# Geo3DSmart/PDANet

Hardware: AMD Instinct MI355X
Metric: scenes/sec (16384-pt ONCE, PDA-SSD forward+backward) (higher is better)
Workload: dtype f32; 1 GPU; once16k_b2_detector_fwd_bwd_adam; scenes_per_gpu=2, global_batch=2, parallelism=dp1, world_size_seen=1, cpu_affinity=GPU-local NUMA node of 0000:dc:00.0: 128 CPUs, full=False, graph_tail=False, graph_head=True

## Files before the change

include/pda_train.h:

```cpp
#ifndef PDA_TRAIN_H
#define PDA_TRAIN_H
#include "pda_pointnet2.h"

#ifdef __cplusplus
extern "C" {
#endif

int pda_grad_norm(const float *g, int64_t n, float *norm_out, float *scratch1024, pda_stream_t stream);
int pda_adam_onecycle_step(float *p, const float *g, float *m, float *v, int64_t n, float lr,
                           float beta1, float beta2, float eps, float wd, int step,
                           const float *total_norm, float max_norm, pda_stream_t stream);

int64_t pda_bn_relu_scratch_bytes(int c);
int pda_bn_relu_fwd(const float *x, const float *gamma, const float *beta, float *running_mean,
                    float *running_var, float *y, float *mean_invstd, void *scratch, int64_t rows, int c,
                    float eps, float momentum, pda_stream_t stream);
int pda_bn_relu_bwd(const float *x, const float *grad_y, const float *gamma, const float *beta,
                    const float *mean_invstd, float *grad_x, float *grad_gamma, float *grad_beta,
                    void *scratch, int64_t rows, int c, pda_stream_t stream);
int pda_bn_relu_fwd_counted(const float *x, const float *gamma, const float *beta, float *running_mean, float *running_var,
                            float *y, float *mean_invstd, void *scratch, int64_t rows, int c, float eps, float momentum,
                            const int32_t *count, int32_t *status, int relu, int training, pda_stream_t stream);
int pda_bn_relu_bwd_counted(const float *x, const float *grad_y, const float *gamma, const float *beta,
                            const float *mean_invstd, float *grad_x, float *grad_gamma, float *grad_beta, void *scratch,
// ... 203 lines not shown
int pda_nms_bev(const float *boxes, const int32_t *num_valid, int64_t *keep, int32_t *num_keep,
                uint64_t *mask_scratch, int b, int n, float thresh, int normal, pda_stream_t stream);
int pda_multi_nms_compact(const float *boxes, const float *scores, const int64_t *keep, const int32_t *num_keep,
                          const int32_t *label_map, int b, int c, int k, int post_max, float *pred_boxes, float *pred_scores,
                          int64_t *pred_labels, int32_t *num_pred, pda_stream_t stream);
int pda_multi_nms_compact_wide(int box_cols, const float *boxes, const float *scores, const int64_t *keep,
                               const int32_t *num_keep, const int32_t *label_map, int b, int c, int k, int post_max,
                               float *pred_boxes, float *pred_scores, int64_t *pred_labels, int32_t *num_pred,
                               pda_stream_t stream);

int pda_head_cls_loss(const float *preds, int row_stride, int col0, int num_class, const int64_t *labels, const float *soft,
                      int64_t n, float scale, float *out2, float *grad, pda_stream_t stream);
int pda_head_centerness(const float *centers, const float *gt, const int64_t *labels, float *out, int64_t n, pda_stream_t stream);
int pda_head_box_loss(const float *preds, const float *labels, const int64_t *cls_labels, const float *code_weights, float beta,
                      int bins, float dir_weight, float box_weight, int64_t n, float *out4, float *grad, pda_stream_t stream);
int pda_head_vote_loss(int mode, const float *origin, const float *offsets, const int64_t *key, const float *gt, int b, int boxes,
                       int num_class, float weight, int64_t n, float *out1, float *grad, pda_stream_t stream);
int pda_head_corner_loss(const float *box_preds, const float *centers, const float *cls_preds, int num_class, const float *gt,
                         const int64_t *cls_labels, const float *mean_size, int bins, float weight, int64_t n, float *out1,
                         float *grad_box, float *grad_centers, pda_stream_t stream);

int64_t pda_sa_small_train_workspace_bytes(void);
int pda_sa_small_train_supported(int c, int nsample, int c1, int c2, int c3, int64_t tokens);
int pda_sa_small_train_fwd(const float *xyz, const float *new_xyz, const float *feat_pm, const int32_t *idx,
                           const float *w1, const float *w2, const float *w3, const float *const *gamma,
                           const float *const *beta, float *const *running_mean, float *const *running_var,
                           const float *eps, const float *momentum, void *workspace, float *out, float *zmax,
                           uint8_t *arg, int b, int n, int m, int c, int nsample, int c1, int c2, int c3,
                           pda_stream_t stream);
int pda_sa_small_train_bwd(const float *xyz, const float *new_xyz, const float *feat_pm, const int32_t *idx,
                           const float *grad_out, const float *zmax, const uint8_t *arg, void *workspace, float *dz2,
                           float *dz1, float *dw1, float *dw2, float *dw3, float *const *dgamma, float *const *dbeta,
                           int b, int n, int m, int c, int nsample, int c1, int c2, int c3, pda_stream_t stream);

int64_t pda_sa_xyz_grad_scratch_bytes(int c1);
int pda_sa_point_gather(const float *point_rows, const float *xyz, const float *new_xyz, const int32_t *idx, const float *w,
                        int ldw, const float *bias, int relu, float *z, int b, int n, int m, int nsample, int c1,
                        pda_stream_t stream);
int pda_sa_xyz_grad(const float *grad_z1, const float *xyz, const float *new_xyz, const int32_t *idx, const float *w, int ldw,
                    float *dw, int lddw, float *grad_new_xyz, void *scratch, int b, int n, int m, int nsample, int c1,
                    pda_stream_t stream);
int64_t pda_sa_point_gather_stats_blocks(int64_t tokens, int c1);
int pda_sa_point_gather_stats(const float *point_rows, const float *xyz, const float *new_xyz, const int32_t *idx,
                              const float *w, int ldw, float *z, double *partial, int b, int n, int m, int nsample, int c1,
                              pda_stream_t stream);
int pda_sa_point_grad_bn(const float *grad_a1, const float *z1, const float *mean_invstd, const float *gamma,
                         const float *beta, const float *bwd_sums, const float *xyz, const float *new_xyz, const int32_t *idx,
                         const float *w, int ldw, float *dw, int lddw, float *grad_new_xyz, float *grad_points, void *scratch,
                         int b, int n, int m, int nsample, int c1, pda_stream_t stream);

int64_t pda_input_stage_workspace_bytes(int batch, int64_t n_cap);
int pda_input_stage(const float *points, const int64_t *offsets, int64_t n_total, int batch, int c, int64_t n_cap,
                    const float *range6, int num_points, const int32_t *pick, const int32_t *perm1, const int32_t *perm2,
                    uint64_t seed, int shuffle, float *out_points, int32_t *info, void *workspace, pda_stream_t stream);
int pda_input_boxes(const float *boxes, const int64_t *box_offsets, int64_t m_total, int batch, int box_dim, int max_gt,
                    const float *range6, int min_num_corners, float *gt_boxes, int32_t *info, pda_stream_t stream);

int64_t pda_augment_workspace_bytes(int batch, int64_t n_cap, int k);
int pda_augment(const float *points, const int64_t *offsets, int64_t n_total, int batch, int c, int64_t n_cap,
                const float *boxes, const int64_t *box_offsets, int64_t m_total, const float *db_points,
                const int64_t *db_offsets, int64_t db_n_points, const float *db_boxes, const double *db_centre,
                const int32_t *db_class, int n_obj, const int32_t *cand, const int32_t *cand_group, const double *cand_dz,
                int k, const int32_t *flip, const double *angle, const float *scale, const float *remove_extra_width,
                int64_t paste_cap, float *out_points, int64_t out_cap, int64_t *out_offsets, float *out_boxes,
                int64_t out_box_cap, int64_t *out_box_offsets, int32_t *info, void *workspace, pda_stream_t stream);

// ... 323 lines not shown
```

pdanet_amd/_lib.py:

```python
import ctypes
import os

_HERE = os.path.dirname(os.path.abspath(__file__))
LIB_PATH = os.environ.get("PDA_LIB_PATH") or os.path.join(_HERE, "libpda_pointnet2.so")
ABI_VERSION = 20


class DensityNetScale(ctypes.Structure):
    _fields_ = [("x", ctypes.c_void_p), ("grad_y", ctypes.c_void_p), ("params", ctypes.c_void_p), ("y", ctypes.c_void_p),
                ("stats", ctypes.c_void_p), ("scratch", ctypes.c_void_p), ("running", ctypes.c_void_p * 6),
                ("grad_params", ctypes.c_void_p), ("n", ctypes.c_int64), ("rowmap", ctypes.c_void_p),
                ("row_weight", ctypes.c_void_p), ("n_unique", ctypes.c_void_p), ("nsample", ctypes.c_int),
                ("eps", ctypes.c_float), ("momentum", ctypes.c_float)]


class OnceFrames(ctypes.Structure):
    _fields_ = [("gt_boxes", ctypes.c_void_p), ("gt_name", ctypes.c_void_p), ("gt_offsets", ctypes.c_void_p),
                ("pred_boxes", ctypes.c_void_p), ("pred_score", ctypes.c_void_p), ("pred_name", ctypes.c_void_p),
                ("pred_start", ctypes.c_void_p), ("pred_count", ctypes.c_void_p), ("iou_start", ctypes.c_void_p),
                ("n_gt_total", ctypes.c_int64), ("pred_cap", ctypes.c_int64), ("iou_cap", ctypes.c_int64),
                ("n_frames", ctypes.c_int), ("max_gt", ctypes.c_int), ("max_pred", ctypes.c_int)]


class KittiFrames(ctypes.Structure):
# ... 105 lines not shown
    "pda_densitynet_param_count": [],
    "pda_densitynet_eval_param_count": [],
    "pda_densitynet_scratch_bytes": [],
    "pda_densitynet_fwd": [_vp, _vp, _vp, _vp, _vp, _vp, _vp, _vp, _vp, _vp, _vp, ctypes.c_int64, _f, _f, _vp],
    "pda_densitynet_bwd": [_vp, _vp, _vp, _vp, _vp, _vp, ctypes.c_int64, _f, _vp],
    "pda_densitynet_eval": [_vp, _vp, _vp, ctypes.c_int64, _vp],
    "pda_densitynet_fwd_multi": [_vp, _i, _vp],
    "pda_densitynet_bwd_multi": [_vp, _i, _vp],
    "pda_densitynet_fwd_unique": [_vp, _vp, _vp, _vp, _vp, _vp, _vp, _vp, _vp, _vp, _vp, ctypes.c_int64, _vp, _vp, _vp, _i, _f, _f, _vp],
    "pda_densitynet_bwd_unique": [_vp, _vp, _vp, _vp, _vp, _vp, ctypes.c_int64, _vp, _vp, _vp, _i, _f, _vp],
    "pda_pda_geometry": [_vp, _vp, _vp, _vp, _vp, _i, _i, _i, _i, _f, _vp],
    "pda_points_in_boxes": [_vp, _vp, _vp, _i, _i, _i, _vp],
    "pda_roiaware_pool3d_fwd": [_vp, _vp, _vp, _vp, _vp, _vp, _i, _i, _i, _i, _i, _i, _i, _i, _vp],
    "pda_roiaware_pool3d_bwd": [_vp, _vp, _vp, _vp, _i, _i, _i, _i, _i, _i, _i, _i, _vp],
    "pda_roipoint_pool3d_fwd": [_vp, _vp, _vp, _vp, _vp, _i, _i, _i, _i, _i, _vp],
    "pda_points_in_boxes_mask": [_vp, _vp, _vp, _i, _i, _vp],
    "pda_points_in_boxes_count": [_vp, _i, _vp, _vp, _i, _i, _i, _vp],
    "pda_assign_point_targets": [_vp, _vp, _vp, _vp, _vp, _vp, _i, _i, _i, _i, _i, _vp],
    "pda_sa_gaussian_mask": [_vp, _i, _i, _vp, _vp, _vp, ctypes.c_int64, _vp],
    "pda_head_assign_targets": [_vp, _i, _i, _vp, ctypes.POINTER(ctypes.c_float), _vp, _vp, _vp, _vp, _vp, _i, _i, _i, _i, _i, _i, _vp],
    "pda_head_cls_loss": [_vp, _i, _i, _i, _vp, _vp, ctypes.c_int64, _f, _vp, _vp, _vp],
    "pda_head_centerness": [_vp, _vp, _vp, _vp, ctypes.c_int64, _vp],
    "pda_head_box_loss": [_vp, _vp, _vp, _vp, _f, _i, _f, _f, ctypes.c_int64, _vp, _vp, _vp],
    "pda_head_vote_loss": [_i, _vp, _vp, _vp, _vp, _i, _i, _i, _f, ctypes.c_int64, _vp, _vp, _vp],
    "pda_head_corner_loss": [_vp, _vp, _vp, _i, _vp, _vp, _vp, _i, _f, ctypes.c_int64, _vp, _vp, _vp, _vp],
    "pda_boxes_overlap_bev": [_vp, _vp, _vp, _i, _i, _vp],
    "pda_boxes_iou_bev": [_vp, _vp, _vp, _i, _i, _vp],
    "pda_nms_mask_words": [_i],
    "pda_nms_bev": [_vp, _vp, _vp, _vp, _vp, _i, _i, _f, _i, _vp],
    "pda_sa_small_train_workspace_bytes": [],
    "pda_sa_small_train_supported": [_i, _i, _i, _i, _i, ctypes.c_int64],
    "pda_sa_small_train_fwd": [_vp] * 7 + [ctypes.POINTER(_vp)] * 4 + [ctypes.POINTER(_f)] * 2 + [_vp] * 4 + [_i] * 8 + [_vp],
    "pda_sa_small_train_bwd": [_vp] * 13 + [ctypes.POINTER(_vp)] * 2 + [_i] * 8 + [_vp],
    "pda_sa_xyz_grad_scratch_bytes": [_i],
    "pda_sa_point_gather": [_vp, _vp, _vp, _vp, _vp, _i, _vp, _i, _vp, _i, _i, _i, _i, _i, _vp],
    "pda_sa_xyz_grad": [_vp, _vp, _vp, _vp, _vp, _i, _vp, _i, _vp, _vp, _i, _i, _i, _i, _i, _vp],
    "pda_sa_point_gather_stats_blocks": [ctypes.c_int64, _i],
    "pda_sa_point_gather_stats": [_vp, _vp, _vp, _vp, _vp, _i, _vp, _vp, _i, _i, _i, _i, _i, _vp],
    "pda_sa_point_grad_bn": [_vp] * 10 + [_i, _vp, _i, _vp, _vp, _vp, _i, _i, _i, _i, _i, _vp],
    "pda_adam_onecycle_step": [_vp, _vp, _vp, _vp, ctypes.c_int64, _f, _f, _f, _f, _f, _i, _vp, _f, _vp],
    "pda_input_stage_workspace_bytes": [_i, ctypes.c_int64],
    "pda_input_stage": [_vp, _vp, ctypes.c_int64, _i, _i, ctypes.c_int64, ctypes.POINTER(_f), _i, _vp, _vp, _vp,
                        ctypes.c_uint64, _i, _vp, _vp, _vp, _vp],
    "pda_input_boxes": [_vp, _vp, ctypes.c_int64, _i, _i, _i, ctypes.POINTER(_f), _i, _vp, _vp, _vp],
    "pda_augment_workspace_bytes": [_i, ctypes.c_int64, _i],
    "pda_augment": [_vp, _vp, ctypes.c_int64, _i, _i, ctypes.c_int64, _vp, _vp, ctypes.c_int64, _vp, _vp, ctypes.c_int64, _vp,
                    _vp, _vp, _i, _vp, _vp, _vp, _i, _vp, _vp, _vp, ctypes.POINTER(_f), ctypes.c_int64, _vp, ctypes.c_int64,
                    _vp, _vp, ctypes.c_int64, _vp, _vp, _vp, _vp],
    "pda_augment_paste": [_vp, _vp, ctypes.c_int64, _i, _i, ctypes.c_int64, _vp, _vp, ctypes.c_int64, _vp, _vp, ctypes.c_int64, _vp,
                          _vp, _vp, _i, _vp, _vp, _vp, _i, ctypes.POINTER(_f), ctypes.c_int64, _vp, ctypes.c_int64, _vp, _vp,
                          ctypes.c_int64, _vp, _vp, _vp, _vp],
    "pda_augment_steps_workspace_bytes": [_i, ctypes.c_int64, _i, _i],
    "pda_augment_steps": [_vp, _vp, ctypes.c_int64, _i, _i, ctypes.c_int64, _vp, _vp, ctypes.c_int64,
                          ctypes.POINTER(ctypes.c_int32), _i, _vp, _vp, _i, _i, _vp, _vp, ctypes.c_int64, _vp, _vp,
                          ctypes.c_int64, _vp, _vp, _vp, _vp],
    "pda_pyramid_aug_workspace_bytes": [_i, ctypes.c_int64, _i],
    "pda_pyramid_aug": [_vp, _vp, ctypes.c_int64, _i, _i, ctypes.c_int64, _vp, _vp, ctypes.c_int64, _vp, _vp, _vp, _vp, _vp, _i,
                        ctypes.POINTER(ctypes.c_double), _i, _i, _i, _vp, _vp, ctypes.c_int64, _vp, _vp, ctypes.c_int64, _vp,
                        _vp, _vp, _vp],
    "pda_once_eval_workspace_bytes": [_i, ctypes.c_int64, _i],
    "pda_once_eval_iou": [ctypes.POINTER(OnceFrames), _i, _vp, _vp, _vp],
    "pda_once_eval_accumulate": [ctypes.POINTER(OnceFrames), _vp, _vp, _i, _i, ctypes.POINTER(ctypes.c_double), _i, _vp, _vp,
                                 _vp, _vp],
    "pda_once_eval_match": [ctypes.POINTER(OnceFrames), _vp, _vp, _i, _i, ctypes.POINTER(ctypes.c_double), _i, _i, _vp, _vp,
                            _vp, _vp, _vp, _vp, _vp, _vp],
    "pda_kitti_eval_workspace_bytes": [_i, ctypes.c_int64, ctypes.c_int64, _i],
# ... 183 lines not shown
```

pdanet_amd/csrc/sa_train_small.hip:

```cpp
#include "pda_common.h"

namespace pda {

typedef float f32x16 __attribute__((ext_vector_type(16)));

constexpr int SS_WAVES = 8;
constexpr int SS_LD = 33;
constexpr int SS_LDS_WAVE = 96 * SS_LD;
constexpr int SS_LDS_WPACK = 6400;
constexpr int SS_LDS_STATE = 768;
__host__ __device__ constexpr int ss_lds_floats(int waves) { return SS_LDS_WPACK + SS_LDS_STATE + waves * SS_LDS_WAVE; }
constexpr int SS_MAX_BLOCKS = 512;
constexpr int SS_PART = 128;
constexpr int SS_DW = 2048;
__host__ __device__ constexpr int ss_state_base(int layer) { return (layer - 1) * 192; }
static_assert(384 + 6 * 64 <= 1024, "the state (floats) fits the first 4 KB of the workspace");
__host__ __device__ constexpr int ss_off_w2() { return 256; }
__host__ __device__ constexpr int ss_off_w3() { return 256 + 1024; }
__host__ __device__ constexpr int ss_off_w2t(int R3) { return 256 + 1024 + 1024 * R3; }
__host__ __device__ constexpr int ss_off_w3t(int R3) { return 256 + 2048 + 1024 * R3; }
__host__ __device__ constexpr int ss_wpack_floats(int R3) { return 256 + 2048 + 2048 * R3; }

struct SsParams {
    const float* xyz;
    const float* new_xyz;
    const float* feat;
    const int32_t* idx;
    const float* wpack;
    const float* state;
    double* partial;
    float* out;
    float* zmax;
    uint8_t* arg;
    const float* gout;
    const uint8_t* arg_in;
    float* dz_out;
    const float* dz_in;
    float* dw_partial;
    int n, m, c, ns, c1, c2, c3;
    int64_t tiles;
};

__device__ __forceinline__ float ss_pack_one(const float* __restrict__ w, int o, int rows, int cols, int R, int mode, int trans) {
    const int e = o & 3, lane = (o >> 2) & 63, rest = o >> 8;
    const int rb = rest % R, tq = rest / R;
    const int t = tq * 4 + e, h = lane >> 5;
    const int row = rb * 32 + (lane & 31);
    int k;
    if (mode == 0) k = 2 * t + h;
    else { const int tt = t & 15; k = 32 * (t >> 4) + (tt & 3) + 8 * (tt >> 2) + 4 * h; }
    if (row >= rows || k >= cols) return 0.f;
    return trans ? w[(size_t)k * rows + row] : w[(size_t)row * cols + k];
}

__global__ void ss_pack_kernel(const float* __restrict__ w1, const float* __restrict__ w2, const float* __restrict__ w3,
                               float* __restrict__ wpack, int c0, int c1, int c2, int c3, int R3) {
    const int total = ss_wpack_floats(R3);
    for (int o = blockIdx.x * blockDim.x + threadIdx.x; o < total; o += gridDim.x * blockDim.x) {
        float v;
        if (o < ss_off_w2()) v = ss_pack_one(w1, o, c1, c0, 1, 0, 0);
        else if (o < ss_off_w3()) v = ss_pack_one(w2, o - ss_off_w2(), c2, c1, 1, 1, 0);
        else if (o < ss_off_w2t(R3)) v = ss_pack_one(w3, o - ss_off_w3(), c3, c2, R3, 1, 0);
        else if (o < ss_off_w3t(R3)) v = ss_pack_one(w2, o - ss_off_w2t(R3), c1, c2, 1, 1, 1);
        else v = ss_pack_one(w3, o - ss_off_w3t(R3), c2, c3, 1, 1, 1);
        wpack[o] = v;
    }
}

template <int KS, int R>
struct SsFrag {
    const float* wf;
    int lane;
    __device__ __forceinline__ void load(const float* lds_wf, int l) { wf = lds_wf; lane = l; }
    __device__ __forceinline__ float4 f(int tq, int r) const { return *reinterpret_cast<const float4*>(wf + ((tq * R + r) * 64 + lane) * 4); }
};

template <int KS, int R, typename HinT>
__device__ __forceinline__ void ss_mm(f32x16 (&acc)[R], const HinT& hin, const SsFrag<KS, R>& w) {
#pragma unroll
    for (int r = 0; r < R; ++r)
#pragma unroll
        for (int i = 0; i < 16; ++i) acc[r][i] = 0.f;
#pragma unroll
    for (int tq = 0; tq < KS / 4; ++tq)
#pragma unroll
        for (int e = 0; e < 4; ++e) {
            const float b = hin(tq * 4 + e);
#pragma unroll
            for (int r = 0; r < R; ++r) {
                const float4 a4 = w.f(tq, r);
// ... 150 lines not shown
    }
}

__device__ __forceinline__ void ss_to_lds(float* __restrict__ t, const f32x16& v, int rb, int lane) {
    const int h = lane >> 5, j = lane & 31;
#pragma unroll
    for (int i = 0; i < 16; ++i) t[(rb * 32 + (i & 3) + 8 * (i >> 2) + 4 * h) * SS_LD + j] = v[i];
}

template <int NB>
__device__ __forceinline__ void ss_dw_tile(f32x16 (&dw)[NB], const float* __restrict__ zt, const float* __restrict__ yt, int lane) {
    const int h = lane >> 5, c = lane & 31;
#pragma unroll
    for (int t = 0; t < 16; ++t) {
        if ((t & 3) == 0) __builtin_amdgcn_sched_barrier(0);
        const float b = yt[c * SS_LD + 2 * t + h];
#pragma unroll
        for (int rb = 0; rb < NB; ++rb)
            dw[rb] = __builtin_amdgcn_mfma_f32_32x32x2f32(zt[(rb * 32 + c) * SS_LD + 2 * t + h], b, dw[rb], 0, 0, 0);
    }
}

__device__ __forceinline__ void ss_wave_fence() { asm volatile("s_waitcnt lgkmcnt(0)" ::: "memory"); }

__device__ __forceinline__ void ss_stage_constants(const SsParams& p, float* smem, int R3) {
    const int nw = ss_wpack_floats(R3);
    for (int e = threadIdx.x * 4; e < nw; e += blockDim.x * 4)
        *reinterpret_cast<float4*>(smem + e) = *reinterpret_cast<const float4*>(p.wpack + e);
    for (int e = threadIdx.x * 4; e < SS_LDS_STATE; e += blockDim.x * 4)
        *reinterpret_cast<float4*>(smem + SS_LDS_WPACK + e) = *reinterpret_cast<const float4*>(p.state + e);
    __syncthreads();
}

template <int R3, int NS, int STAGE, int W>
__global__ __launch_bounds__(W * 64) void ss_fwd_kernel(const SsParams p) {
    extern __shared__ __attribute__((aligned(16))) float smem[];
    const int w = wave_id(), lane = lane_id(), h = lane >> 5, j = lane & 31;
    float* lds_all = smem + SS_LDS_WPACK + SS_LDS_STATE;
    float* lds = lds_all + w * SS_LDS_WAVE;
    ss_stage_constants(p, smem, R3);
    SsFrag<4, 1> w1;
    SsFrag<16, 1> w2;
    SsFrag<16, R3> w3;
    w1.load(smem, lane);
    w2.load(smem + ss_off_w2(), lane);
    w3.load(smem + ss_off_w3(), lane);
    const float* st1 = smem + SS_LDS_WPACK + ss_state_base(1);
    const float* st2 = smem + SS_LDS_WPACK + ss_state_base(2);
    const float* st3 = smem + SS_LDS_WPACK + ss_state_base(3);
    constexpr int NB = STAGE == 3 ? R3 : 1;
    double s1[NB][16], s2[NB][16];
#pragma unroll
    for (int b = 0; b < NB; ++b)
#pragma unroll
        for (int i = 0; i < 16; ++i) { s1[b][i] = 0.0; s2[b][i] = 0.0; }
    const int ech = lane % p.c3, eg = lane / p.c3;
    float emu = 0.f, eis = 0.f, ega = 0.f, ebe = 0.f;
    if (STAGE == 4) { emu = st3[ech]; eis = st3[32 * R3 + ech]; ega = st3[64 * R3 + ech]; ebe = st3[96 * R3 + ech]; }

    SsWalk walk;
    walk.start(p, (int64_t)blockIdx.x * W + w, (int64_t)gridDim.x * W, j, h);
    for (; walk.tile < p.tiles; walk.tile += walk.stride) {
        const int64_t tile = walk.tile;
        asm volatile("" ::: "memory");
        float x0[4];
        walk.fetch(p, j, h, x0);
        f32x16 a1[1], a2[1], a3[R3], dummy;
        ss_mm<4, 1>(a1, SsX0{x0}, w1);
        if (STAGE == 1) {
#pragma unroll
            for (int i = 0; i < 16; ++i) { const double z = a1[0][i]; s1[0][i] += z; s2[0][i] += z * z; }
            continue;
        }
        ss_bn_relu<false>(a1[0], dummy, st1, 32, 0, h);
        ss_mm<16, 1>(a2, SsAcc<1>{a1}, w2);
        if (STAGE == 2) {
#pragma unroll
            for (int i = 0; i < 16; ++i) { const double z = a2[0][i]; s1[0][i] += z; s2[0][i] += z * z; }
            continue;
        }
        ss_bn_relu<false>(a2[0], dummy, st2, 32, 0, h);
        ss_mm<16, R3>(a3, SsAcc<1>{a2}, w3);
        if (STAGE == 3) {
#pragma unroll
            for (int b = 0; b < NB; ++b)
#pragma unroll
                for (int i = 0; i < 16; ++i) { const double z = a3[b][i]; s1[b][i] += z; s2[b][i] += z * z; }
            continue;
        }
#pragma unroll
        for (int rb = 0; rb < R3; ++rb) ss_to_lds(lds, a3[rb], rb, lane);
        ss_wave_fence();
        float best = -1.f, bz = 0.f;
        int bs = 0;
        const float* zrow = lds + ech * SS_LD + eg * NS;
#pragma unroll 8
        for (int s = 0; s < NS; ++s) {
            const float z = zrow[s];
            const float y = fmaxf((z - emu) * eis * ega + ebe, 0.f);
            if (y > best) { best = y; bz = z; bs = s; }
        }
        p.out[tile * 64 + lane] = best;
        p.zmax[tile * 64 + lane] = bz;
        p.arg[tile * 64 + lane] = (uint8_t)bs;
        ss_wave_fence();
    }
    if (STAGE <= 3) ss_store_partial<NB, W, double>(s1, s2, p.partial + (size_t)blockIdx.x * SS_PART, lds_all);
}

__global__ __launch_bounds__(256) void ss_pool_sums_kernel(const float* __restrict__ gout, const float* __restrict__ zmax,
                                                           const float* __restrict__ st3, int P3, int c3, int64_t groups,
                                                           double* __restrict__ partial) {
    __shared__ double red[2][256][4];
    const int cg = c3 / 4, col = threadIdx.x % cg, r0 = threadIdx.x / cg, rpb = 256 / cg;
    const float4 mu = *reinterpret_cast<const float4*>(st3 + 4 * col), is = *reinterpret_cast<const float4*>(st3 + P3 + 4 * col);
    const float4 ga = *reinterpret_cast<const float4*>(st3 + 2 * P3 + 4 * col), be = *reinterpret_cast<const float4*>(st3 + 3 * P3 + 4 * col);
    double a[4] = {0, 0, 0, 0}, b[4] = {0, 0, 0, 0};
    for (int64_t g = (int64_t)blockIdx.x * rpb + r0; g < groups; g += (int64_t)gridDim.x * rpb) {
        const float4 go = *reinterpret_cast<const float4*>(gout + g * c3 + 4 * col);
        const float4 z = *reinterpret_cast<const float4*>(zmax + g * c3 + 4 * col);
#pragma unroll
        for (int e = 0; e < 4; ++e) {
            const float xh = (f4(z, e) - f4(mu, e)) * f4(is, e);
            const float dyh = (xh * f4(ga, e) + f4(be, e) > 0.f) ? f4(go, e) : 0.f;
            a[e] += dyh;
            b[e] += (double)dyh * xh;
        }
    }
#pragma unroll
    for (int e = 0; e < 4; ++e) { red[0][threadIdx.x][e] = a[e]; red[1][threadIdx.x][e] = b[e]; }
    __syncthreads();
    double* part = partial + (size_t)blockIdx.x * SS_PART;
    if (threadIdx.x < 128) {
        const int which = threadIdx.x >> 6, ch = threadIdx.x & 63;
        double s = 0.0;
        if (ch < c3)
            for (int r = 0; r < rpb; ++r) s += red[which][r * cg + ch / 4][ch & 3];
        part[threadIdx.x] = s;
    }
}
// ... 127 lines not shown
            float* row = p.dz_out + tok * cdn;
#pragma unroll
            for (int q = 0; q < 4; ++q) {
                float o[4];
#pragma unroll
                for (int e = 0; e < 4; ++e) {
                    o[e] = y[4 * q + e] > 0.f ? d[0][4 * q + e] : 0.f;
                    s1[0][4 * q + e] += o[e];
                    s2[0][4 * q + e] += o[e] * xh[4 * q + e];
                }
                if (8 * q + 4 * h < cdn) *reinterpret_cast<float4*>(row + 8 * q + 4 * h) = make_float4(o[0], o[1], o[2], o[3]);
            }
        }
    }
    if (STAGE >= 2) ss_store_partial<1, W, float>(s1, s2, p.partial + (size_t)blockIdx.x * SS_PART, lds_all);
    ss_store_dw<NBW, W>(dw, p.dw_partial + (size_t)blockIdx.x * SS_DW, lds_all);
}

__device__ __forceinline__ bool ss_sum_partials(const double* __restrict__ partial, int nblocks, double& a, double& b, int& ch) {
    __shared__ double red[2][16][64];
    ch = threadIdx.x & 63;
    const int part = threadIdx.x >> 6;
    double x = 0.0, y = 0.0;
    for (int k = part; k < nblocks; k += 16) { x += partial[(size_t)k * SS_PART + ch]; y += partial[(size_t)k * SS_PART + 64 + ch]; }
    red[0][part][ch] = x; red[1][part][ch] = y;
    __syncthreads();
    if (part != 0) return false;
    a = 0.0; b = 0.0;
#pragma unroll
    for (int q = 0; q < 16; ++q) { a += red[0][q][ch]; b += red[1][q][ch]; }
    return true;
}

__global__ __launch_bounds__(1024) void ss_finalize_fwd_kernel(const double* __restrict__ partial, int nblocks, int c, int P,
                                                                int64_t rows, float eps, float momentum,
                                                                const float* __restrict__ gamma, const float* __restrict__ beta,
                                                                float* __restrict__ st, float* __restrict__ running_mean,
                                                                float* __restrict__ running_var) {
    double s1, s2;
    int ch;
    if (!ss_sum_partials(partial, nblocks, s1, s2, ch) || ch >= P) return;
    if (ch >= c) {
        st[ch] = 0.f; st[P + ch] = 0.f; st[2 * P + ch] = 0.f; st[3 * P + ch] = 0.f;
        return;
    }
    const double mean = s1 / (double)rows;
    double var = s2 / (double)rows - mean * mean;
    var = var < 0 ? 0 : var;
    st[ch] = (float)mean;
    st[P + ch] = (float)(1.0 / sqrt(var + (double)eps));
    st[2 * P + ch] = gamma[ch];
    st[3 * P + ch] = beta[ch];
    if (running_mean) {
        const double unbiased = rows > 1 ? var * ((double)rows / (double)(rows - 1)) : var;
        running_mean[ch] = (float)((1.0 - momentum) * running_mean[ch] + momentum * mean);
        running_var[ch] = (float)((1.0 - momentum) * running_var[ch] + momentum * unbiased);
    }
}

__global__ __launch_bounds__(1024) void ss_finalize_bwd_kernel(const double* __restrict__ partial, int nblocks, int c, int P, int64_t rows,
                                                                float* __restrict__ st, float* __restrict__ dgamma, float* __restrict__ dbeta,
                                                                const float* __restrict__ dw_partial, int dw_blocks, int dw_rows, int dw_cols,
                                                                float* __restrict__ dw) {
    if (blockIdx.x == 0) {
        if (partial == nullptr) return;
        double s1, s2;
        int ch;
        if (!ss_sum_partials(partial, nblocks, s1, s2, ch) || ch >= P) return;
        st[4 * P + ch] = ch < c ? (float)(s1 / (double)rows) : 0.f;
        st[5 * P + ch] = ch < c ? (float)(s2 / (double)rows) : 0.f;
        if (ch < c) { dbeta[ch] = (float)s1; dgamma[ch] = (float)s2; }
        return;
    }
    __shared__ double red[16][64];
    const int el = threadIdx.x & 63, part = threadIdx.x >> 6;
    const int e = (blockIdx.x - 1) * 64 + el;
    const bool ok = dw != nullptr && e < dw_rows * dw_cols;
    const int row = ok ? e / dw_cols : 0, col = ok ? e % dw_cols : 0;
    double a = 0.0;
    if (ok)
        for (int k = part; k < dw_blocks; k += 16) a += (double)dw_partial[(size_t)k * SS_DW + row * 32 + col];
    red[part][el] = a;
    __syncthreads();
    if (part == 0 && ok) {
        double t = 0.0;
#pragma unroll
        for (int q = 0; q < 16; ++q) t += red[q][el];
        dw[e] = (float)t;
    }
}

template <typename K>
static bool ss_lds_ok(K kern, PerDevice<bool>& once, int bytes) {
    return once.get([kern, bytes] { return hipFuncSetAttribute((const void*)kern, hipFuncAttributeMaxDynamicSharedMemorySize, bytes) == hipSuccess; });
}
static int ss_blocks_for(int64_t tiles, int waves) {
    const int64_t want = divup64(tiles, waves);
    return (int)(want < 256 ? want : 256);
}

template <int R3, int NS, int STAGE>
static bool ss_launch_fwd_stage(const SsParams& p, hipStream_t s, int& blocks) {
    constexpr int W = SS_WAVES;
    static PerDevice<bool> once;
    constexpr int bytes = ss_lds_floats(W) * (int)sizeof(float);
    if (!ss_lds_ok(ss_fwd_kernel<R3, NS, STAGE, W>, once, bytes)) return false;
    blocks = ss_blocks_for(p.tiles, W);
    hipLaunchKernelGGL((ss_fwd_kernel<R3, NS, STAGE, W>), dim3(blocks), dim3(W * 64), bytes, s, p);
    return true;
}
template <int R3, int NS>
static bool ss_launch_fwd(int stage, const SsParams& p, hipStream_t s, int& blocks) {
    switch (stage) {
        case 1: return ss_launch_fwd_stage<R3, NS, 1>(p, s, blocks);
        case 2: return ss_launch_fwd_stage<R3, NS, 2>(p, s, blocks);
        case 3: return ss_launch_fwd_stage<R3, NS, 3>(p, s, blocks);
        default: return ss_launch_fwd_stage<R3, NS, 4>(p, s, blocks);
    }
}
template <int R3, int NS, int STAGE>
static bool ss_launch_bwd_stage(const SsParams& p, hipStream_t s, int& blocks) {
    constexpr int W = SS_WAVES;
    static PerDevice<bool> once;
    constexpr int bytes = ss_lds_floats(W) * (int)sizeof(float);
    if (!ss_lds_ok(ss_bwd_kernel<R3, NS, STAGE, W>, once, bytes)) return false;
    blocks = ss_blocks_for(p.tiles, W);
    hipLaunchKernelGGL((ss_bwd_kernel<R3, NS, STAGE, W>), dim3(blocks), dim3(W * 64), bytes, s, p);
    return true;
}
template <int R3, int NS>
static bool ss_launch_bwd(int stage, const SsParams& p, hipStream_t s, int& blocks) {
    switch (stage) {
        case 3: return ss_launch_bwd_stage<R3, NS, 3>(p, s, blocks);
        case 2: return ss_launch_bwd_stage<R3, NS, 2>(p, s, blocks);
        default: return ss_launch_bwd_stage<R3, NS, 1>(p, s, blocks);
    }
}

static int ss_check_shape(const char* what, int b, int n, int m, int c, int ns, int c1, int c2, int c3) {
    PDA_REQUIRE(b >= 1 && n >= 1 && m >= 1, "%s: bad size (b=%d n=%d m=%d)", what, b, n, m);
    const bool ok = c >= 0 && c <= 5 && (ns == 16 || ns == 32) && (c1 == 16 || c1 == 32) && (c2 == 16 || c2 == 32) &&
                    (c3 == 32 || c3 == 64) && (32 / ns) * c3 == 64 && ((int64_t)b * m * ns) % 32 == 0;
    if (!ok) {
        set_error("%s: no kernel built for the chain %d -> %d -> %d -> %d over %d neighbours (built: 3 + c <= 8 inputs, "
                  "widths 16 | 32, 16 | 32, and (nsample, c3) = (16, 32) | (32, 64))", what, 3 + c, c1, c2, c3, ns);
        return PDA_ERR_UNSUPPORTED;
    }
    return PDA_OK;
}

constexpr size_t SS_WS_STATE = 0;
constexpr size_t SS_WS_WPACK = 4096;
constexpr size_t SS_WS_PARTIAL = SS_WS_WPACK + 32768;
constexpr size_t SS_WS_DW = SS_WS_PARTIAL + (size_t)SS_MAX_BLOCKS * SS_PART * sizeof(double);
constexpr size_t SS_WS_BYTES = SS_WS_DW + (size_t)SS_MAX_BLOCKS * SS_DW * sizeof(float);

}

PDA_API int64_t pda_sa_small_train_workspace_bytes(void) { return (int64_t)pda::SS_WS_BYTES; }

PDA_API int pda_sa_small_train_supported(int c, int ns, int c1, int c2, int c3, int64_t tokens) {
    return c >= 0 && c <= 5 && (ns == 16 || ns == 32) && (c1 == 16 || c1 == 32) && (c2 == 16 || c2 == 32) && (c3 == 32 || c3 == 64) &&
           (32 / ns) * c3 == 64 && tokens > 0 && tokens % 32 == 0;
}

PDA_API int pda_sa_small_train_fwd(const float* xyz, const float* new_xyz, const float* feat_pm, const int32_t* idx, const float* w1,
                                   const float* w2, const float* w3, const float* const* gamma, const float* const* beta,
                                   float* const* running_mean, float* const* running_var, const float* eps, const float* momentum,
                                   void* workspace, float* out, float* zmax, uint8_t* arg, int b, int n, int m, int c, int ns, int c1,
                                   int c2, int c3, pda_stream_t stream) {
    using namespace pda;
    const int rc = ss_check_shape("pda_sa_small_train_fwd", b, n, m, c, ns, c1, c2, c3);
    if (rc != PDA_OK) return rc;
    PDA_REQUIRE(xyz && new_xyz && idx && w1 && w2 && w3 && gamma && beta && running_mean && running_var && eps && momentum && workspace &&
                out && zmax && arg && (feat_pm || c == 0), "pda_sa_small_train_fwd: null pointer");
    PDA_REQUIRE(((uintptr_t)workspace & 255) == 0, "pda_sa_small_train_fwd: workspace must be 256-byte aligned");
    const hipStream_t s = (hipStream_t)stream;
    char* ws = (char*)workspace;
    float* state = (float*)(ws + SS_WS_STATE);
    float* wpack = (float*)(ws + SS_WS_WPACK);
    const int R3 = c3 / 32;
    hipLaunchKernelGGL(ss_pack_kernel, dim3(8), dim3(256), 0, s, w1, w2, w3, wpack, 3 + c, c1, c2, c3, R3);
    SsParams p{};
    p.xyz = xyz; p.new_xyz = new_xyz; p.feat = feat_pm; p.idx = idx; p.wpack = wpack; p.state = state;
    p.partial = (double*)(ws + SS_WS_PARTIAL); p.out = out; p.zmax = zmax; p.arg = arg;
    p.n = n; p.m = m; p.c = c; p.ns = ns; p.c1 = c1; p.c2 = c2; p.c3 = c3;
    const int64_t tokens = (int64_t)b * m * ns;
    p.tiles = tokens / 32;
    int blocks = 0;
    const int cs[3] = {c1, c2, c3}, Ps[3] = {32, 32, 32 * R3};
    for (int stage = 1; stage <= 4; ++stage) {
        const bool ok = R3 == 1 ? ss_launch_fwd<1, 16>(stage, p, s, blocks) : ss_launch_fwd<2, 32>(stage, p, s, blocks);
        PDA_REQUIRE(ok, "pda_sa_small_train_fwd: dynamic LDS refused");
        if (stage <= 3)
            hipLaunchKernelGGL(ss_finalize_fwd_kernel, dim3(1), dim3(1024), 0, s, (const double*)p.partial, blocks, cs[stage - 1],
                               Ps[stage - 1], tokens, eps[stage - 1], momentum[stage - 1], gamma[stage - 1], beta[stage - 1],
                               state + ss_state_base(stage), running_mean[stage - 1], running_var[stage - 1]);
    }
    return check_launch("pda_sa_small_train_fwd");
}

PDA_API int pda_sa_small_train_bwd(const float* xyz, const float* new_xyz, const float* feat_pm, const int32_t* idx, const float* grad_out,
                                   const float* zmax, const uint8_t* arg, void* workspace, float* dz2, float* dz1, float* dw1, float* dw2,
                                   float* dw3, float* const* dgamma, float* const* dbeta, int b, int n, int m, int c, int ns, int c1,
                                   int c2, int c3, pda_stream_t stream) {
    using namespace pda;
    const int rc = ss_check_shape("pda_sa_small_train_bwd", b, n, m, c, ns, c1, c2, c3);
    if (rc != PDA_OK) return rc;
    PDA_REQUIRE(xyz && new_xyz && idx && grad_out && zmax && arg && workspace && dz2 && dz1 && dw1 && dw2 && dw3 && dgamma && dbeta &&
                (feat_pm || c == 0), "pda_sa_small_train_bwd: null pointer");
    const hipStream_t s = (hipStream_t)stream;
    char* ws = (char*)workspace;
    float* state = (float*)(ws + SS_WS_STATE);
    SsParams p{};
    p.xyz = xyz; p.new_xyz = new_xyz; p.feat = feat_pm; p.idx = idx; p.wpack = (const float*)(ws + SS_WS_WPACK); p.state = state;
    p.partial = (double*)(ws + SS_WS_PARTIAL); p.dw_partial = (float*)(ws + SS_WS_DW);
    p.gout = grad_out; p.arg_in = arg;
    p.n = n; p.m = m; p.c = c; p.ns = ns; p.c1 = c1; p.c2 = c2; p.c3 = c3;
    const int64_t tokens = (int64_t)b * m * ns, groups = (int64_t)b * m;
    p.tiles = tokens / 32;
    int blocks = 0;
    const int R3 = c3 / 32;
    const int pb = (int)(divup64(groups, 256 / (c3 / 4)) < 256 ? divup64(groups, 256 / (c3 / 4)) : 256);
    hipLaunchKernelGGL(ss_pool_sums_kernel, dim3(pb), dim3(256), 0, s, grad_out, zmax, (const float*)(state + ss_state_base(3)), 32 * R3, c3,
                       groups, p.partial);
    hipLaunchKernelGGL(ss_finalize_bwd_kernel, dim3(1), dim3(1024), 0, s, (const double*)p.partial, pb, c3, 32 * R3, tokens,
                       state + ss_state_base(3), dgamma[2], dbeta[2], (const float*)nullptr, 0, 0, 0, (float*)nullptr);
    p.dz_out = dz2;
// ... 17 lines not shown
```

Before: 124.4 scenes/s.

## Distribute SA small-train forward tiles via atomic work-claiming units with per-unit stat partials

Replaces the static grid-stride tile walk in the fused SA forward kernel with dynamic work units claimed through a global atomic counter, using a small LDS ring and prefetching tile indices three steps ahead. BN statistics are folded per unit into partial rows, and the finalize kernel now reduces many more rows across multiple workgroups instead of one. Gather uses per-scene tile arithmetic when possible. The aim is better load balance across CUs and more latency hiding, at the cost of extra atomics, per-unit syncs and partial-row traffic. A debug setter allows overriding unit sizes.

```diff
diff --git a/include/pda_train.h b/include/pda_train.h
--- a/include/pda_train.h
+++ b/include/pda_train.h
@@ -259,6 +259,7 @@
                            const float *grad_out, const float *zmax, const uint8_t *arg, void *workspace, float *dz2,
                            float *dz1, float *dw1, float *dw2, float *dw3, float *const *dgamma, float *const *dbeta,
                            int b, int n, int m, int c, int nsample, int c1, int c2, int c3, pda_stream_t stream);
+int pda_sa_small_train_set_sharing(int max_workgroups, int unit_stats, int unit_pool);
 
 int64_t pda_sa_xyz_grad_scratch_bytes(int c1);
 int pda_sa_point_gather(const float *point_rows, const float *xyz, const float *new_xyz, const int32_t *idx, const float *w,
diff --git a/pdanet_amd/_lib.py b/pdanet_amd/_lib.py
--- a/pdanet_amd/_lib.py
+++ b/pdanet_amd/_lib.py
@@ -161,6 +161,7 @@
     "pda_sa_small_train_supported": [_i, _i, _i, _i, _i, ctypes.c_int64],
     "pda_sa_small_train_fwd": [_vp] * 7 + [ctypes.POINTER(_vp)] * 4 + [ctypes.POINTER(_f)] * 2 + [_vp] * 4 + [_i] * 8 + [_vp],
     "pda_sa_small_train_bwd": [_vp] * 13 + [ctypes.POINTER(_vp)] * 2 + [_i] * 8 + [_vp],
+    "pda_sa_small_train_set_sharing": [_i, _i, _i],
     "pda_sa_xyz_grad_scratch_bytes": [_i],
     "pda_sa_point_gather": [_vp, _vp, _vp, _vp, _vp, _i, _vp, _i, _vp, _i, _i, _i, _i, _i, _vp],
     "pda_sa_xyz_grad": [_vp, _vp, _vp, _vp, _vp, _i, _vp, _i, _vp, _vp, _i, _i, _i, _i, _i, _vp],
diff --git a/pdanet_amd/csrc/sa_train_small.hip b/pdanet_amd/csrc/sa_train_small.hip
--- a/pdanet_amd/csrc/sa_train_small.hip
+++ b/pdanet_amd/csrc/sa_train_small.hip
@@ -1,4 +1,6 @@
 #include "pda_common.h"
+
+#include <atomic>
 
 namespace pda {
 
@@ -11,6 +13,17 @@
 constexpr int SS_LDS_STATE = 768;
 __host__ __device__ constexpr int ss_lds_floats(int waves) { return SS_LDS_WPACK + SS_LDS_STATE + waves * SS_LDS_WAVE; }
 constexpr int SS_MAX_BLOCKS = 512;
+constexpr int SS_CUS = 256;
+constexpr int SS_MAX_UNITS = 4096;
+#ifndef SS_STATS_UNITS_PER_CU
+#define SS_STATS_UNITS_PER_CU 4
+#endif
+#ifndef SS_POOL_UNITS_PER_CU
+#define SS_POOL_UNITS_PER_CU 8
+#endif
+constexpr int SS_UNITS_STATS = SS_STATS_UNITS_PER_CU;
+constexpr int SS_UNITS_POOL = SS_POOL_UNITS_PER_CU;
+constexpr int SS_RING = 8;
 constexpr int SS_PART = 128;
 constexpr int SS_DW = 2048;
 __host__ __device__ constexpr int ss_state_base(int layer) { return (layer - 1) * 192; }
@@ -39,6 +52,10 @@
     float* dw_partial;
     int n, m, c, ns, c1, c2, c3;
     int64_t tiles;
+    int* counter;
+    int64_t units;
+    int unit;
+    int tps;
 };
 
 __device__ __forceinline__ float ss_pack_one(const float* __restrict__ w, int o, int rows, int cols, int R, int mode, int trans) {
@@ -54,8 +71,9 @@
 }
 
 __global__ void ss_pack_kernel(const float* __restrict__ w1, const float* __restrict__ w2, const float* __restrict__ w3,
-                               float* __restrict__ wpack, int c0, int c1, int c2, int c3, int R3) {
+                               float* __restrict__ wpack, int* __restrict__ counters, int c0, int c1, int c2, int c3, int R3) {
     const int total = ss_wpack_floats(R3);
+    if (blockIdx.x == 0 && threadIdx.x < 4) counters[threadIdx.x] = 0;
     for (int o = blockIdx.x * blockDim.x + threadIdx.x; o < total; o += gridDim.x * blockDim.x) {
         float v;
         if (o < ss_off_w2()) v = ss_pack_one(w1, o, c1, c0, 1, 0, 0);
@@ -272,12 +290,95 @@
     __syncthreads();
 }
 
+template <int NS>
+__device__ __forceinline__ void ss_gather_tile(const SsParams& p, int64_t tile, int j, int id, int h, float (&x0)[4]) {
+    if (p.tps == 0) { ss_gather(p, tile * 32 + j, id, h, x0); return; }
+    const unsigned t = (unsigned)tile, bs = t / (unsigned)p.tps;
+    const int centre = (int)(((t - bs * (unsigned)p.tps) * 32u + (unsigned)j) / (unsigned)NS);
+    const float* pt = p.xyz + ((size_t)bs * p.n + id) * 3;
+    const float* ct = p.new_xyz + ((size_t)bs * p.m + centre) * 3;
+    const float dx = pt[0] - ct[0], dy = pt[1] - ct[1], dz = pt[2] - ct[2];
+    const float* f = p.feat ? p.feat + ((size_t)bs * p.n + id) * p.c : nullptr;
+    x0[0] = h == 0 ? dx : dy;
+    x0[1] = h == 0 ? dz : ((f && 0 < p.c) ? f[0] : 0.f);
+#pragma unroll
+    for (int t2 = 2; t2 < 4; ++t2) {
+        const int ch = 2 * t2 + h - 3;
+        x0[t2] = (f && ch < p.c) ? f[ch] : 0.f;
+    }
+}
+
+__device__ __forceinline__ int ss_claim(int* counter, int k) {
+    return counter ? atomicAdd(counter, 1) : (k == 0 ? (int)blockIdx.x : 0x7fffffff);
+}
+
+struct SsClaims {
+    const int* ring;
+    int64_t tiles, units;
+    int U, w;
+    __device__ __forceinline__ int64_t tile_of(int q, int i) const {
+        const int u = __builtin_amdgcn_readfirstlane(ring[q & (SS_RING - 1)]);
+        const int64_t t = ((int64_t)u * U + i) * SS_WAVES + w;
+        return (u < units && t < tiles) ? t : -1;
+    }
+};
+
+template <int NS>
+struct SsUnitWalk {
+    int64_t cur, a1, a2;
+    int id1, id2;
+    float xn[4];
+    __device__ __forceinline__ void start(const SsParams& p, int64_t t0, int64_t t1, int64_t t2, int j, int h) {
+        cur = t0; a1 = t1; a2 = t2;
+        const int id0 = p.idx[(t0 < 0 ? 0 : t0) * 32 + j];
+        id1 = p.idx[(t1 < 0 ? 0 : t1) * 32 + j];
+        id2 = p.idx[(t2 < 0 ? 0 : t2) * 32 + j];
+        ss_gather_tile<NS>(p, t0 < 0 ? 0 : t0, j, id0, h, xn);
+    }
+    __device__ __forceinline__ void fetch(const SsParams& p, int j, int h, float (&x0)[4], int64_t t3) {
+#pragma unroll
+        for (int t = 0; t < 4; ++t) x0[t] = xn[t];
+        ss_gather_tile<NS>(p, a1 < 0 ? 0 : a1, j, id1, h, xn);
+        id1 = id2;
+        id2 = p.idx[(t3 < 0 ? 0 : t3) * 32 + j];
+        cur = a1; a1 = a2; a2 = t3;
+    }
+};
+
+template <int NB>
+__device__ __forceinline__ void ss_fold_unit(const double (&s1)[NB][16], const double (&s2)[NB][16], float* lds_wave, int parity, int lane) {
+    double* buf = reinterpret_cast<double*>(lds_wave);
+    double* wsum = buf + 1024 + parity * 128;
+    const int o = lane & 31, t = lane >> 5, i = o >> 1, hh = o & 1;
+    const int chl = (i & 3) + 8 * (i >> 2) + 4 * hh;
+#pragma unroll
+    for (int b = 0; b < NB; ++b)
+#pragma unroll
+        for (int which = 0; which < 2; ++which) {
+            ss_wave_fence();
+#pragma unroll
+            for (int r = 0; r < 16; ++r) buf[r * 64 + lane] = which ? s2[b][r] : s1[b][r];
+            ss_wave_fence();
+            double a = 0.0;
+#pragma unroll
+            for (int k = 0; k < 16; ++k) a += buf[i * 64 + hh * 32 + t * 16 + ((k + o) & 15)];
+            a += __shfl_xor(a, 32);
+            if (t == 0) wsum[which * 64 + b * 32 + chl] = a;
+        }
+}
+static_assert(1024 + 2 * 128 <= SS_LDS_WAVE / 2, "the exchange block and both sum blocks fit a wave's tile area");
+
 template <int R3, int NS, int STAGE, int W>
 __global__ __launch_bounds__(W * 64) void ss_fwd_kernel(const SsParams p) {
     extern __shared__ __attribute__((aligned(16))) float smem[];
-    const int w = wave_id(), lane = lane_id(), h = lane >> 5, j = lane & 31;
+    __shared__ int ring[SS_RING];
+    const int w = __builtin_amdgcn_readfirstlane(wave_id()), lane = lane_id(), h = lane >> 5, j = lane & 31;
     float* lds_all = smem + SS_LDS_WPACK + SS_LDS_STATE;
     float* lds = lds_all + w * SS_LDS_WAVE;
+    const int U = p.unit, D = 1 + 2 / U;
+    int pending = 0;
+    if (threadIdx.x == 0)
+        for (int k = 0; k <= D; ++k) ring[k] = ss_claim(p.counter, k);
     ss_stage_constants(p, smem, R3);
     SsFrag<4, 1> w1;
     SsFrag<16, 1> w2;
@@ -298,13 +399,20 @@
     float emu = 0.f, eis = 0.f, ega = 0.f, ebe = 0.f;
     if (STAGE == 4) { emu = st3[ech]; eis = st3[32 * R3 + ech]; ega = st3[64 * R3 + ech]; ebe = st3[96 * R3 + ech]; }
 
-    SsWalk walk;
-    walk.start(p, (int64_t)blockIdx.x * W + w, (int64_t)gridDim.x * W, j, h);
-    for (; walk.tile < p.tiles; walk.tile += walk.stride) {
-        const int64_t tile = walk.tile;
+    const SsClaims cl{ring, p.tiles, p.units, U, w};
+    int q = 0, parity = 0;
+    int q3 = 3 / U, i3 = 3 % U;
+    SsUnitWalk<NS> walk;
+    walk.start(p, cl.tile_of(0, 0), cl.tile_of(1 / U, 1 % U), cl.tile_of(2 / U, 2 % U), j, h);
+    for (int ucur = __builtin_amdgcn_readfirstlane(ring[0]); ucur < p.units; ucur = __builtin_amdgcn_readfirstlane(ring[q & (SS_RING - 1)])) {
+      for (int i = 0; i < U; ++i) {
+        const int64_t tile = walk.cur;
+        if (i == U - 1 && threadIdx.x == 0) pending = ss_claim(p.counter, q + D + 1);
         asm volatile("" ::: "memory");
         float x0[4];
-        walk.fetch(p, j, h, x0);
+        walk.fetch(p, j, h, x0, cl.tile_of(q3, i3));
+        if (++i3 == U) { i3 = 0; ++q3; }
+        if (tile < 0) continue;
         f32x16 a1[1], a2[1], a3[R3], dummy;
         ss_mm<4, 1>(a1, SsX0{x0}, w1);
         if (STAGE == 1) {
@@ -344,8 +452,24 @@
         p.zmax[tile * 64 + lane] = bz;
         p.arg[tile * 64 + lane] = (uint8_t)bs;
         ss_wave_fence();
-    }
-    if (STAGE <= 3) ss_store_partial<NB, W, double>(s1, s2, p.partial + (size_t)blockIdx.x * SS_PART, lds_all);
+      }
+      if (STAGE <= 3) ss_fold_unit<NB>(s1, s2, lds, parity, lane);
+      if (threadIdx.x == 0) ring[(q + D + 1) & (SS_RING - 1)] = pending;
+      __syncthreads();
+      if (STAGE <= 3) {
+        if (threadIdx.x < 128 && (threadIdx.x & 63) < 32 * NB) {
+            double a = 0.0;
+#pragma unroll
+            for (int ww = 0; ww < W; ++ww) a += reinterpret_cast<const double*>(lds_all + ww * SS_LDS_WAVE)[1024 + parity * 128 + threadIdx.x];
+            p.partial[(size_t)ucur * SS_PART + threadIdx.x] = a;
+        }
+#pragma unroll
+        for (int b = 0; b < NB; ++b)
+#pragma unroll
+            for (int r = 0; r < 16; ++r) { s1[b][r] = 0.0; s2[b][r] = 0.0; }
+      }
+      ++q; parity ^= 1;
+    }
 }
 
 __global__ __launch_bounds__(256) void ss_pool_sums_kernel(const float* __restrict__ gout, const float* __restrict__ zmax,
@@ -539,6 +663,30 @@
     return true;
 }
 
+__device__ __forceinline__ bool ss_sum_unit_rows(const double* __restrict__ partial, int nrows, double& a, double& b, int& ch) {
+    __shared__ double red[2][128][8];
+    __shared__ double red2[2][16][8];
+    const int c = threadIdx.x & 7, slice = threadIdx.x >> 3;
+    ch = blockIdx.x * 8 + c;
+    double x = 0.0, y = 0.0;
+#pragma unroll 4
+    for (int k = slice; k < nrows; k += 128) { x += partial[(size_t)k * SS_PART + ch]; y += partial[(size_t)k * SS_PART + 64 + ch]; }
+    red[0][slice][c] = x; red[1][slice][c] = y;
+    __syncthreads();
+    if (slice < 16) {
+        x = 0.0; y = 0.0;
+#pragma unroll
+        for (int k = 0; k < 8; ++k) { x += red[0][slice * 8 + k][c]; y += red[1][slice * 8 + k][c]; }
+        red2[0][slice][c] = x; red2[1][slice][c] = y;
+    }
+    __syncthreads();
+    if (slice != 0) return false;
+    a = 0.0; b = 0.0;
+#pragma unroll
+    for (int k = 0; k < 16; ++k) { a += red2[0][k][c]; b += red2[1][k][c]; }
+    return true;
+}
+
 __global__ __launch_bounds__(1024) void ss_finalize_fwd_kernel(const double* __restrict__ partial, int nblocks, int c, int P,
                                                                 int64_t rows, float eps, float momentum,
                                                                 const float* __restrict__ gamma, const float* __restrict__ beta,
@@ -546,7 +694,7 @@
                                                                 float* __restrict__ running_var) {
     double s1, s2;
     int ch;
-    if (!ss_sum_partials(partial, nblocks, s1, s2, ch) || ch >= P) return;
+    if (!ss_sum_unit_rows(partial, nblocks, s1, s2, ch) || ch >= P) return;
     if (ch >= c) {
         st[ch] = 0.f; st[P + ch] = 0.f; st[2 * P + ch] = 0.f; st[3 * P + ch] = 0.f;
         return;
@@ -606,18 +754,33 @@
     return (int)(want < 256 ? want : 256);
 }
 
+static std::atomic<int> ss_dbg_cap{0}, ss_dbg_unit_stats{0}, ss_dbg_unit_pool{0};
+
+static int ss_plan_fwd(SsParams& p, int stage) {
+    const int cap_set = ss_dbg_cap.load(), cap = cap_set > 0 && cap_set < SS_CUS ? cap_set : SS_CUS;
+    const int set = stage <= 3 ? ss_dbg_unit_stats.load() : ss_dbg_unit_pool.load();
+    int64_t u = set > 0 ? set : (set < 0 ? divup64(p.tiles, (int64_t)SS_WAVES * cap)
+                                         : p.tiles / ((int64_t)SS_WAVES * SS_CUS * (stage <= 3 ? SS_UNITS_STATS : SS_UNITS_POOL)));
+    if (u < 1) u = 1;
+    if (set < 0) p.counter = nullptr;
+    if (stage <= 3 && u < divup64(p.tiles, (int64_t)SS_WAVES * SS_MAX_UNITS)) u = divup64(p.tiles, (int64_t)SS_WAVES * SS_MAX_UNITS);
+    if (u < divup64(p.tiles, (int64_t)SS_WAVES << 30)) u = divup64(p.tiles, (int64_t)SS_WAVES << 30);
+    p.unit = (int)u;
+    p.units = divup64(p.tiles, (int64_t)SS_WAVES * u);
+    return (int)(p.units < cap ? p.units : cap);
+}
+
 template <int R3, int NS, int STAGE>
-static bool ss_launch_fwd_stage(const SsParams& p, hipStream_t s, int& blocks) {
+static bool ss_launch_fwd_stage(const SsParams& p, hipStream_t s, int blocks) {
     constexpr int W = SS_WAVES;
     static PerDevice<bool> once;
     constexpr int bytes = ss_lds_floats(W) * (int)sizeof(float);
     if (!ss_lds_ok(ss_fwd_kernel<R3, NS, STAGE, W>, once, bytes)) return false;
-    blocks = ss_blocks_for(p.tiles, W);
     hipLaunchKernelGGL((ss_fwd_kernel<R3, NS, STAGE, W>), dim3(blocks), dim3(W * 64), bytes, s, p);
     return true;
 }
 template <int R3, int NS>
-static bool ss_launch_fwd(int stage, const SsParams& p, hipStream_t s, int& blocks) {
+static bool ss_launch_fwd(int stage, const SsParams& p, hipStream_t s, int blocks) {
     switch (stage) {
         case 1: return ss_launch_fwd_stage<R3, NS, 1>(p, s, blocks);
         case 2: return ss_launch_fwd_stage<R3, NS, 2>(p, s, blocks);
@@ -659,12 +822,21 @@
 constexpr size_t SS_WS_STATE = 0;
 constexpr size_t SS_WS_WPACK = 4096;
 constexpr size_t SS_WS_PARTIAL = SS_WS_WPACK + 32768;
-constexpr size_t SS_WS_DW = SS_WS_PARTIAL + (size_t)SS_MAX_BLOCKS * SS_PART * sizeof(double);
-constexpr size_t SS_WS_BYTES = SS_WS_DW + (size_t)SS_MAX_BLOCKS * SS_DW * sizeof(float);
+static_assert(SS_MAX_UNITS >= SS_MAX_BLOCKS, "the partial rows serve the forward units and the backward workgroups");
+constexpr size_t SS_WS_DW = SS_WS_PARTIAL + (size_t)SS_MAX_UNITS * SS_PART * sizeof(double);
+constexpr size_t SS_WS_COUNTERS = SS_WS_DW + (size_t)SS_MAX_BLOCKS * SS_DW * sizeof(float);
+constexpr size_t SS_WS_BYTES = SS_WS_COUNTERS + 256;
 
 }
 
 PDA_API int64_t pda_sa_small_train_workspace_bytes(void) { return (int64_t)pda::SS_WS_BYTES; }
+
+PDA_API int pda_sa_small_train_set_sharing(int max_workgroups, int unit_stats, int unit_pool) {
+    pda::ss_dbg_cap.store(max_workgroups);
+    pda::ss_dbg_unit_stats.store(unit_stats);
+    pda::ss_dbg_unit_pool.store(unit_pool);
+    return PDA_OK;
+}
 
 PDA_API int pda_sa_small_train_supported(int c, int ns, int c1, int c2, int c3, int64_t tokens) {
     return c >= 0 && c <= 5 && (ns == 16 || ns == 32) && (c1 == 16 || c1 == 32) && (c2 == 16 || c2 == 32) && (c3 == 32 || c3 == 64) &&
@@ -687,20 +859,24 @@
     float* state = (float*)(ws + SS_WS_STATE);
     float* wpack = (float*)(ws + SS_WS_WPACK);
     const int R3 = c3 / 32;
-    hipLaunchKernelGGL(ss_pack_kernel, dim3(8), dim3(256), 0, s, w1, w2, w3, wpack, 3 + c, c1, c2, c3, R3);
+    int* counters = (int*)(ws + SS_WS_COUNTERS);
+    hipLaunchKernelGGL(ss_pack_kernel, dim3(8), dim3(256), 0, s, w1, w2, w3, wpack, counters, 3 + c, c1, c2, c3, R3);
     SsParams p{};
     p.xyz = xyz; p.new_xyz = new_xyz; p.feat = feat_pm; p.idx = idx; p.wpack = wpack; p.state = state;
     p.partial = (double*)(ws + SS_WS_PARTIAL); p.out = out; p.zmax = zmax; p.arg = arg;
     p.n = n; p.m = m; p.c = c; p.ns = ns; p.c1 = c1; p.c2 = c2; p.c3 = c3;
     const int64_t tokens = (int64_t)b * m * ns;
     p.tiles = tokens / 32;
-    int blocks = 0;
+    const int64_t per_scene = (int64_t)m * ns;
+    p.tps = per_scene % 32 == 0 && tokens < ((int64_t)1 << 31) ? (int)(per_scene / 32) : 0;
     const int cs[3] = {c1, c2, c3}, Ps[3] = {32, 32, 32 * R3};
     for (int stage = 1; stage <= 4; ++stage) {
+        p.counter = counters + (stage - 1);
+        const int blocks = ss_plan_fwd(p, stage);
         const bool ok = R3 == 1 ? ss_launch_fwd<1, 16>(stage, p, s, blocks) : ss_launch_fwd<2, 32>(stage, p, s, blocks);
         PDA_REQUIRE(ok, "pda_sa_small_train_fwd: dynamic LDS refused");
         if (stage <= 3)
-            hipLaunchKernelGGL(ss_finalize_fwd_kernel, dim3(1), dim3(1024), 0, s, (const double*)p.partial, blocks, cs[stage - 1],
+            hipLaunchKernelGGL(ss_finalize_fwd_kernel, dim3(Ps[stage - 1] / 8), dim3(1024), 0, s, (const double*)p.partial, (int)p.units, cs[stage - 1],
                                Ps[stage - 1], tokens, eps[stage - 1], momentum[stage - 1], gamma[stage - 1], beta[stage - 1],
                                state + ss_state_base(stage), running_mean[stage - 1], running_var[stage - 1]);
     }
```

Result: no change. 124.2 scenes/s (-0.2%).
